# HengyiWang/spann3r

Measured on NVIDIA H100. Metric: frames/sec (512x384, 10-frame seq) enc->mem-attn->dec->DPT, higher is better.
Workload: dtype bf16x3 (split-bf16 operands, fp32 accumulate; tf32 attention)

## Files before the change

### include/spann3r_b200.h

```cpp
#ifndef SPANN3R_B200_H_
#define SPANN3R_B200_H_

#include <stddef.h>
#include <stdint.h>

#ifdef __cplusplus
extern "C" {
#endif

#define S3R_VERSION 100

enum { S3R_EPI_PLAIN = 0, S3R_EPI_PIXSHUF = 1, S3R_EPI_QKV = 2, S3R_EPI_HEADTAIL = 3 };
enum { S3R_ACT_NONE = 0, S3R_ACT_GELU = 1, S3R_ACT_RELU = 2 };

int s3r_version(void);
int s3r_abi_sizeof(int which );
const char* s3r_last_error(void);
int s3r_device_ok(void);


int s3r_split(const float* x, int64_t ldx, void* hi, void* lo, int64_t ldp, int col0, int64_t rows, int c, int relu,
              void* stream);

int s3r_layernorm(const float* x, int64_t ldx, const float* w, const float* b, int64_t wb_group_stride,
                  int64_t rows_per_group, float eps, int64_t rows, int c, float* out, int64_t ldo, void* hi, void* lo,
                  int64_t ldp, int col0, int64_t swap_rows, void* stream);

int s3r_rope2d_inplace(float* tokens, const int64_t* pos, int64_t bn, int h, int d, int64_t stride_tok,
                       int64_t stride_head, float base, float fwd, void* stream);

int s3r_im2col_patch16(const float* img, int64_t sb, int64_t sc, int64_t sy, int64_t sx, int b, int gh, int gw,
                       void* hi, void* lo, void* stream);
int s3r_im2col_3x3s2(const void* ihi, const void* ilo, int nb, int h, int w, int c, int ho, int wo, void* ohi,
                     void* olo, void* stream);
int s3r_upsample2x(const float* x, int nb, int h, int w, int c, float* out, void* hi, void* lo, void* stream);

size_t s3r_conv_wgrad_workspace_bytes(int nb, int h, int w, int n, int kc, int taps);
int s3r_conv_wgrad(const void* dy_hi, const void* dy_lo, int64_t ldy, const void* x_hi, const void* x_lo, int64_t ldx,
                   int nb, int h, int w, int n, int kc, int taps, void* workspace, size_t workspace_bytes, float* dw,
                   void* stream);
int s3r_col2im_3x3s2(const float* cols, int nb, int h, int w, int c, int ho, int wo, float* out, void* stream);

typedef struct s3r_gemm_desc {
  const void* a_hi; const void* a_lo;
  const void* b_hi; const void* b_lo;
  int groups, nb, h, w, kc, taps, n;
  int epi, act, plane_relu, force_bn;
  const float* bias;
  const float* res1; int64_t ldr1;
  const float* res2; int64_t ldr2;
  float* out_f32; int64_t ldo;
  void* out_hi; void* out_lo; int64_t ldp; int plane_col0;
  int ps_s, ps_cout;
  int q_c, q_role_base, q_ntok, q_ntok_pad, q_rope, q_nb;
  const int32_t* q_pos; const float* q_cs;
  float* q_out; float* k_out; float* vt_out; float q_scale;
  const float* ht_w; const float* ht_b; float* ht_pts; float* ht_conf;
  const float* ln_stats; int ln_np; float ln_eps; const float* ln_cs; int a_swap;
  float* stats_out;
  uint64_t* trace;
  int swap_col0; float* k2_out; float* vt2_out;
  int precision;
} s3r_gemm_desc;
int s3r_gemm(const s3r_gemm_desc* d, void* stream);
int s3r_gemm_tile_n(const s3r_gemm_desc* d);

int s3r_attention(const float* q, const float* k, const float* vt, int bh, int heads, int nq, int nk, int nk_pad,
                  void* o_hi, void* o_lo, float* o_f32, int64_t ldo, void* stream);

int s3r_conf_score(const float* conf, int64_t n, float* scratch256, float* out, void* stream);
int s3r_conf_score_batched(const float* conf, int batch, int64_t hw, float* scratch, float* out, void* stream);

int s3r_resample_h_u8(const uint8_t* src, int64_t row_stride, int rows, int out_cols, const int32_t* bounds,
                      const int32_t* kk, int ksize, int max_span, uint8_t* dst, void* stream);
int s3r_resample_v_u8_norm(const uint8_t* tmp, int cols, int out_rows, const int32_t* bounds, const int32_t* kk, int ksize,
                           float* dst, void* stream);

int s3r_focal_weiszfeld(const float* pts3d, int b, int h, int w, float ppx, float ppy, int iters, float lo, float hi,
                        float* scratch, float* focal, void* stream);

int s3r_focal_median(const float* pts3d, int b, int h, int w, float ppx, float ppy, float lo, float hi, int32_t* scratch,
                     float* focal, void* stream);

size_t s3r_pnp_workspace_bytes(int b, int n_samples);
int s3r_pnp_ransac(const float* pts3d, const float* img_pts, int b, int64_t n, int width, double fx, double fy, double cx,
                   double cy, float reproj_err, int n_samples, int refine_iters, uint64_t seed, void* workspace,
                   double* out, uint8_t* inlier_mask, void* stream);

size_t s3r_pcl_index_bytes(int64_t n);
int s3r_pcl_index_build(const void* pts, int is_f64, int64_t n, const double* transform, void* index, void* stream);
int s3r_pcl_nearest(const void* index, int64_t n, const void* queries, int is_f64, int64_t nq, const double* transform,
                    double max_dist, double* dist, int64_t* idx, void* stream);
int s3r_pcl_normals(const void* index, int64_t n, int k, double* normals, void* stream);
size_t s3r_pcl_icp_workspace_bytes(void);
int s3r_pcl_icp(const void* source, int is_f64, int64_t ns, const void* target_index, int64_t nt,
                double max_correspondence_distance, const double* init, int max_iteration, double relative_fitness,
                double relative_rmse, void* workspace, double* out, void* stream);
size_t s3r_pcl_stats_workspace_bytes(void);
int s3r_pcl_stats(const double* x, int64_t n, double threshold, void* workspace, double* out, void* stream);
int s3r_pcl_abs_dot(const double* a, const double* b, const int64_t* idx, int64_t n, double* out, void* stream);

size_t s3r_render_workspace_bytes(int width, int height);
int s3r_render_clear(void* keys, int width, int height, void* stream);
int s3r_render_splat(const float* pts, const uint8_t* mask, int64_t n, int64_t id0, const double* camera, double z_near,
                     int width, int height, void* keys, void* stream);
int s3r_render_resolve(const void* keys, const float* colors, int width, int height, uint8_t* rgb, void* stream);

typedef struct s3r_loss_desc {
  int frames, batch, height, width;
  int norm_mode, gt_scale, fix_first, shift_inv, scale_inv, conf_loss, has_dist_clip;
  float alpha, dist_clip;
  const float* pose0;
  const float* const* gt_pts;
  const uint8_t* const* valid;
  const float* const* pred;
  const float* const* conf;
} s3r_loss_desc;
#define S3R_LOSS_RES_HEADER 20
#define S3R_LOSS_RES_PER_B 6
size_t s3r_loss_workspace_bytes(const s3r_loss_desc* d);
int s3r_loss_forward(const s3r_loss_desc* d, void* workspace, size_t workspace_bytes, float* gt_out, float* pred_out,
// ... 99 lines not shown
```

### spann3r_b200/_lib.py

```python
from __future__ import annotations

import ctypes as C
import os

import torch

_HERE = os.path.dirname(os.path.abspath(__file__))
LIB_PATH = os.environ.get("S3R_LIB", os.path.join(_HERE, "libspann3r_b200.so"))

EPI_PLAIN, EPI_PIXSHUF, EPI_QKV, EPI_HEADTAIL = 0, 1, 2, 3
PRECISION_SPLIT, PRECISION_BF16 = 0, 1
ACT_NONE, ACT_GELU, ACT_RELU = 0, 1, 2

_vp, _i, _i64, _f = C.c_void_p, C.c_int, C.c_int64, C.c_float


class GemmDesc(C.Structure):
    _fields_ = [
        ("a_hi", _vp), ("a_lo", _vp), ("b_hi", _vp), ("b_lo", _vp),
        ("groups", _i), ("nb", _i), ("h", _i), ("w", _i), ("kc", _i), ("taps", _i), ("n", _i),
        ("epi", _i), ("act", _i), ("plane_relu", _i), ("force_bn", _i),
        ("bias", _vp),
        ("res1", _vp), ("ldr1", _i64),
        ("res2", _vp), ("ldr2", _i64),
        ("out_f32", _vp), ("ldo", _i64),
        ("out_hi", _vp), ("out_lo", _vp), ("ldp", _i64), ("plane_col0", _i),
        ("ps_s", _i), ("ps_cout", _i),
        ("q_c", _i), ("q_role_base", _i), ("q_ntok", _i), ("q_ntok_pad", _i), ("q_rope", _i), ("q_nb", _i),
        ("q_pos", _vp), ("q_cs", _vp),
        ("q_out", _vp), ("k_out", _vp), ("vt_out", _vp), ("q_scale", _f),
        ("ht_w", _vp), ("ht_b", _vp), ("ht_pts", _vp), ("ht_conf", _vp),
        ("ln_stats", _vp), ("ln_np", _i), ("ln_eps", _f), ("ln_cs", _vp), ("a_swap", _i),
        ("stats_out", _vp),
        ("trace", _vp),
        ("swap_col0", _i), ("k2_out", _vp), ("vt2_out", _vp),
        ("precision", _i),
    ]


class LossDesc(C.Structure):
    _fields_ = [
        ("frames", _i), ("batch", _i), ("height", _i), ("width", _i),
        ("norm_mode", _i), ("gt_scale", _i), ("fix_first", _i), ("shift_inv", _i), ("scale_inv", _i), ("conf_loss", _i),
        ("has_dist_clip", _i), ("alpha", _f), ("dist_clip", _f),
        ("pose0", _vp), ("gt_pts", C.POINTER(_vp)), ("valid", C.POINTER(_vp)), ("pred", C.POINTER(_vp)),
        ("conf", C.POINTER(_vp)),
    ]


LOSS_RES_HEADER, LOSS_RES_PER_B = 20, 6


class AttnTrainDesc(C.Structure):
    _fields_ = [
        ("batch", _i), ("heads", _i), ("nq", _i), ("nk", _i), ("dh", _i), ("scale", _f),
        ("q", _vp), ("k", _vp), ("v", _vp),
        ("q_stride", _i64 * 3), ("k_stride", _i64 * 3), ("v_stride", _i64 * 3),
    ]

_PROTOS = {
    "s3r_version": (_i, []),
    "s3r_abi_sizeof": (_i, [_i]),
    "s3r_last_error": (C.c_char_p, []),
    "s3r_device_ok": (_i, []),
    "s3r_split": (_i, [_vp, _i64, _vp, _vp, _i64, _i, _i64, _i, _i, _vp]),
    "s3r_layernorm": (_i, [_vp, _i64, _vp, _vp, _i64, _i64, _f, _i64, _i, _vp, _i64, _vp, _vp, _i64, _i, _i64, _vp]),
    "s3r_rope2d_inplace": (_i, [_vp, _vp, _i64, _i, _i, _i64, _i64, _f, _f, _vp]),
    "s3r_im2col_patch16": (_i, [_vp, _i64, _i64, _i64, _i64, _i, _i, _i, _vp, _vp, _vp]),
    "s3r_im2col_3x3s2": (_i, [_vp, _vp, _i, _i, _i, _i, _i, _i, _vp, _vp, _vp]),
    "s3r_upsample2x": (_i, [_vp, _i, _i, _i, _i, _vp, _vp, _vp, _vp]),
    "s3r_conv_wgrad_workspace_bytes": (C.c_size_t, [_i, _i, _i, _i, _i, _i]),
    "s3r_conv_wgrad": (_i, [_vp, _vp, _i64, _vp, _vp, _i64, _i, _i, _i, _i, _i, _i, _vp, C.c_size_t, _vp, _vp]),
    "s3r_col2im_3x3s2": (_i, [_vp, _i, _i, _i, _i, _i, _i, _vp, _vp]),
    "s3r_gemm": (_i, [C.POINTER(GemmDesc), _vp]),
    "s3r_gemm_tile_n": (_i, [C.POINTER(GemmDesc)]),
    "s3r_attention": (_i, [_vp, _vp, _vp, _i, _i, _i, _i, _i, _vp, _vp, _vp, _i64, _vp]),
    "s3r_conf_score": (_i, [_vp, _i64, _vp, _vp, _vp]),
    "s3r_conf_score_batched": (_i, [_vp, _i, _i64, _vp, _vp, _vp]),
    "s3r_dropout_mask": (_i, [_vp, _i64, C.c_uint64, _f, _vp]),
    "s3r_set_option": (_i, [C.c_char_p, _i]),
    "s3r_focal_weiszfeld": (_i, [_vp, _i, _i, _i, _f, _f, _i, _f, _f, _vp, _vp, _vp]),
    "s3r_focal_median": (_i, [_vp, _i, _i, _i, _f, _f, _f, _f, _vp, _vp, _vp]),
    "s3r_pnp_workspace_bytes": (C.c_size_t, [_i, _i]),
    "s3r_pnp_ransac": (_i, [_vp, _vp, _i, _i64, _i, C.c_double, C.c_double, C.c_double, C.c_double, _f, _i, _i, C.c_uint64,
                            _vp, _vp, _vp, _vp]),
    "s3r_pcl_index_bytes": (C.c_size_t, [_i64]),
    "s3r_pcl_index_build": (_i, [_vp, _i, _i64, _vp, _vp, _vp]),
    "s3r_pcl_nearest": (_i, [_vp, _i64, _vp, _i, _i64, _vp, C.c_double, _vp, _vp, _vp]),
    "s3r_pcl_normals": (_i, [_vp, _i64, _i, _vp, _vp]),
    "s3r_pcl_icp_workspace_bytes": (C.c_size_t, []),
    "s3r_pcl_icp": (_i, [_vp, _i, _i64, _vp, _i64, C.c_double, _vp, _i, C.c_double, C.c_double, _vp, _vp, _vp]),
    "s3r_pcl_stats_workspace_bytes": (C.c_size_t, []),
    "s3r_pcl_stats": (_i, [_vp, _i64, C.c_double, _vp, _vp, _vp]),
    "s3r_pcl_abs_dot": (_i, [_vp, _vp, _vp, _i64, _vp, _vp]),
    "s3r_render_workspace_bytes": (C.c_size_t, [_i, _i]),
    "s3r_render_clear": (_i, [_vp, _i, _i, _vp]),
    "s3r_render_splat": (_i, [_vp, _vp, _i64, _i64, _vp, C.c_double, _i, _i, _vp, _vp]),
    "s3r_render_resolve": (_i, [_vp, _vp, _i, _i, _vp, _vp]),
    "s3r_loss_workspace_bytes": (C.c_size_t, [C.POINTER(LossDesc)]),
    "s3r_loss_forward": (_i, [C.POINTER(LossDesc), _vp, C.c_size_t, _vp, _vp, _vp, _vp, _vp]),
    "s3r_loss_backward": (_i, [C.POINTER(LossDesc), _vp, C.c_size_t, _vp, _vp, _vp, _vp]),
    "s3r_attn_train_workspace_bytes": (C.c_size_t, [C.POINTER(AttnTrainDesc)]),
    "s3r_attn_train_forward": (_i, [C.POINTER(AttnTrainDesc), _vp, _vp, _vp]),
    "s3r_attn_train_backward": (_i, [C.POINTER(AttnTrainDesc), _vp, _vp, _vp, _vp, C.c_size_t, _vp, _vp, _vp, _vp]),
    "s3r_resample_h_u8": (_i, [_vp, _i64, _i, _i, _vp, _vp, _i, _i, _vp, _vp]),
    "s3r_resample_v_u8_norm": (_i, [_vp, _i, _i, _vp, _vp, _i, _vp, _vp]),
}

_lib = None


class S3RError(RuntimeError):
    pass


def lib():
    global _lib
    if _lib is None:
        if not os.path.exists(LIB_PATH):
            raise S3RError(f"{LIB_PATH} not found: run `python -m spann3r_b200.build` "
                           "(the package has no CPU / eager fallback)")
        L = C.CDLL(LIB_PATH)
        for name, (res, args) in _PROTOS.items():
            fn = getattr(L, name)
            fn.restype = res
            fn.argtypes = args
        _ENGINE_PROTOS_HOOK(L)
        _lib = L
    return _lib
# ... 162 lines not shown
```

### spann3r_b200/csrc/attention.cu

```cuda
#include "common.cuh"
#include "kernels.cuh"
#include "wgmma.cuh"

#include <cstdlib>
#include <cstring>

namespace s3r {

namespace attn {
constexpr int BQ = 128;
constexpr int BKV = 128;
constexpr int D = 64;
constexpr int Q_BYTES = BQ * D * 4;
constexpr int K_BYTES = BKV * D * 4;
constexpr int V_BYTES = D * BKV * 4;
constexpr int KV_STAGES = 3;
constexpr int SMEM = Q_BYTES + KV_STAGES * (K_BYTES + V_BYTES) + 1024 + 256;
constexpr int kThreads = 384;
constexpr int kConsumerWarps = 8;
}

__global__ void __launch_bounds__(attn::kThreads, 1) attention_kernel(const __grid_constant__ AttnArgs args) {
  using namespace attn;
  extern __shared__ uint8_t smem_raw[];
  uint8_t* smem = smem_raw + ((1024u - (smem_u32(smem_raw) & 1023u)) & 1023u);
  uint8_t* sQ = smem;
  uint8_t* sKV = sQ + Q_BYTES;
  uint64_t* bars = reinterpret_cast<uint64_t*>(sKV + KV_STAGES * (K_BYTES + V_BYTES));
  uint64_t* q_full = bars;
  uint64_t* kv_full = bars + 1;
  uint64_t* kv_empty = bars + 1 + KV_STAGES;

  const int warp = threadIdx.x >> 5, lane = threadIdx.x & 31;
  const int q0 = blockIdx.x * BQ;
  const int bh = blockIdx.y;
  const int nblk = (args.nk + BKV - 1) / BKV;

  if (warp == 0 && lane == 0) {
    tma_prefetch_desc(&args.tmQ);
    tma_prefetch_desc(&args.tmK);
    tma_prefetch_desc(&args.tmV);
    mbar_init(q_full, 1);
    for (int i = 0; i < KV_STAGES; ++i) {
      mbar_init(&kv_full[i], 1);
      mbar_init(&kv_empty[i], kConsumerWarps);
    }
    fence_barrier_init();
  }
  __syncthreads();
  pdl_launch_dependents();
  pdl_wait();

  if (warp < 4) {
    asm volatile("setmaxnreg.dec.sync.aligned.u32 40;");
    if (warp == 0 && lane == 0) {
      mbar_arrive_expect_tx(q_full, Q_BYTES);
      tma_load_3d(sQ, &args.tmQ, q_full, 0, q0, bh);
      tma_load_3d(sQ + Q_BYTES / 2, &args.tmQ, q_full, 32, q0, bh);
      for (int j = 0; j < nblk; ++j) {
        const int st = j % KV_STAGES;
        const uint32_t ph = (j / KV_STAGES) & 1;
        mbar_wait(&kv_empty[st], ph ^ 1);
        uint8_t* k = sKV + st * (K_BYTES + V_BYTES);
        uint8_t* v = k + K_BYTES;
        mbar_arrive_expect_tx(&kv_full[st], K_BYTES + V_BYTES);
        tma_load_3d(k, &args.tmK, &kv_full[st], 0, j * BKV, bh);
        tma_load_3d(k + K_BYTES / 2, &args.tmK, &kv_full[st], 32, j * BKV, bh);
#pragma unroll
        for (int a = 0; a < 4; ++a) tma_load_3d(v + a * (V_BYTES / 4), &args.tmV, &kv_full[st], j * BKV + a * 32, 0, bh);
      }
    }
    return;
  }

  asm volatile("setmaxnreg.inc.sync.aligned.u32 232;");
  const int wg = (warp - 4) >> 2;
  const int wq = warp & 3;
  const int g = lane >> 2, t4 = lane & 3;
  const uint32_t aQ = __shfl_sync(0xffffffffu, smem_u32(sQ), 0) + wg * (64 * 128);
  const uint32_t aKV = __shfl_sync(0xffffffffu, smem_u32(sKV), 0);
  constexpr float kLog2e = 1.4426950408889634f;

  float o[32];
#pragma unroll
  for (int i = 0; i < 32; ++i) o[i] = 0.f;
  float m0 = -INFINITY, m1 = -INFINITY, l0 = 0.f, l1 = 0.f;
  const int src_lo = (lane & ~3) | (t4 >> 1), src_hi = src_lo + 2;
  const bool odd = (t4 & 1) != 0;

  mbar_wait(q_full, 0);
  for (int j = 0; j < nblk; ++j) {
    const int st = j % KV_STAGES;
    mbar_wait(&kv_full[st], (j / KV_STAGES) & 1);
    const uint32_t aK = aKV + st * (K_BYTES + V_BYTES);
    const uint32_t aV = aK + K_BYTES;

    float s[64];
    wgmma_fence();
#pragma unroll
    for (int kk = 0; kk < 8; ++kk) {
      const uint32_t part = (kk >> 2) * (Q_BYTES / 2), ko = (kk & 3) * 2;
      wgmma_tf32_n128_ss(s, wgmma_desc_sw128_kmajor(aQ + part) + ko, wgmma_desc_sw128_kmajor(aK + part) + ko, kk > 0);
    }
    wgmma_commit();
    wgmma_wait<0>();

    const int kbase = j * BKV;
    if (kbase + BKV > args.nk) {
#pragma unroll
      for (int i = 0; i < 16; ++i) {
        const int c = kbase + 8 * i + 2 * t4;
        if (c >= args.nk) { s[4 * i] = -INFINITY; s[4 * i + 2] = -INFINITY; }
        if (c + 1 >= args.nk) { s[4 * i + 1] = -INFINITY; s[4 * i + 3] = -INFINITY; }
      }
    }
    float b0 = -INFINITY, b1 = -INFINITY;
#pragma unroll
    for (int i = 0; i < 16; ++i) {
      b0 = fmaxf(b0, fmaxf(s[4 * i], s[4 * i + 1]));
      b1 = fmaxf(b1, fmaxf(s[4 * i + 2], s[4 * i + 3]));
    }
#pragma unroll
    for (int x = 1; x < 4; x <<= 1) {
      b0 = fmaxf(b0, __shfl_xor_sync(0xffffffffu, b0, x));
      b1 = fmaxf(b1, __shfl_xor_sync(0xffffffffu, b1, x));
    }
    const float n0 = fmaxf(m0, b0), n1 = fmaxf(m1, b1);
    const float al0 = (j == 0) ? 0.f : exp2f((m0 - n0) * kLog2e);
    const float al1 = (j == 0) ? 0.f : exp2f((m1 - n1) * kLog2e);
    m0 = n0;
    m1 = n1;
    const float nr0 = -n0 * kLog2e, nr1 = -n1 * kLog2e;
    float ps0 = 0.f, ps1 = 0.f;
#pragma unroll
    for (int i = 0; i < 64; ++i) {
      const bool r1 = (i & 2) != 0;
      const float e = exp2f(fmaf(s[i], kLog2e, r1 ? nr1 : nr0));
      const uint32_t rb = (__float_as_uint(e) + 0x1000u) & 0xffffe000u;
      s[i] = __uint_as_float(rb);
      if (r1) ps1 += s[i]; else ps0 += s[i];
    }
    l0 = l0 * al0 + ps0;
    l1 = l1 * al1 + ps1;
#pragma unroll
    for (int i = 0; i < 8; ++i) {
      o[4 * i] *= al0; o[4 * i + 1] *= al0;
      o[4 * i + 2] *= al1; o[4 * i + 3] *= al1;
    }

    uint32_t pa[16][4];
#pragma unroll
    for (int kk = 0; kk < 16; ++kk) {
      const float x0 = __shfl_sync(0xffffffffu, s[4 * kk], src_lo), x1 = __shfl_sync(0xffffffffu, s[4 * kk + 1], src_lo);
      const float y0 = __shfl_sync(0xffffffffu, s[4 * kk + 2], src_lo), y1 = __shfl_sync(0xffffffffu, s[4 * kk + 3], src_lo);
      const float z0 = __shfl_sync(0xffffffffu, s[4 * kk], src_hi), z1 = __shfl_sync(0xffffffffu, s[4 * kk + 1], src_hi);
      const float w0 = __shfl_sync(0xffffffffu, s[4 * kk + 2], src_hi), w1 = __shfl_sync(0xffffffffu, s[4 * kk + 3], src_hi);
      pa[kk][0] = __float_as_uint(odd ? x1 : x0);
      pa[kk][1] = __float_as_uint(odd ? y1 : y0);
      pa[kk][2] = __float_as_uint(odd ? z1 : z0);
      pa[kk][3] = __float_as_uint(odd ? w1 : w0);
    }
    wgmma_fence();
#pragma unroll
    for (int kk = 0; kk < 16; ++kk)
      wgmma_tf32_n64_rs(o, pa[kk], wgmma_desc_sw128_kmajor(aV + (kk >> 2) * (V_BYTES / 4)) + (kk & 3) * 2, 1);
    wgmma_commit();
    wgmma_wait<0>();
    __syncwarp();
    if (lane == 0) mbar_arrive(&kv_empty[st]);
  }

#pragma unroll
  for (int x = 1; x < 4; x <<= 1) {
    l0 += __shfl_xor_sync(0xffffffffu, l0, x);
    l1 += __shfl_xor_sync(0xffffffffu, l1, x);
  }
  const float inv0 = 1.0f / l0, inv1 = 1.0f / l1;
  const int b = bh / args.heads, h = bh - b * args.heads;
#pragma unroll
  for (int r = 0; r < 2; ++r) {
    const int q = q0 + wg * 64 + wq * 16 + g + 8 * r;
    if (q >= args.nq) continue;
    const float inv = r ? inv1 : inv0;
    const long long row = ((long long)b * args.nq + q) * args.ldo + h * D;
#pragma unroll
    for (int i = 0; i < 8; ++i) {
      const float x = o[4 * i + 2 * r] * inv, y = o[4 * i + 2 * r + 1] * inv;
      const long long off = row + 8 * i + 2 * t4;
      if (args.o_f32) *reinterpret_cast<float2*>(args.o_f32 + off) = make_float2(x, y);
      if (args.o_hi) {
        uint32_t hh, ll;
        split2_bf16(x, y, hh, ll);
        *reinterpret_cast<uint32_t*>(args.o_hi + off) = hh;
        *reinterpret_cast<uint32_t*>(args.o_lo + off) = ll;
      }
    }
  }
}

int attn_plan_init(AttnPlan* plan, const float* q, const float* k, const float* vt, int BH, int heads, int nq, int nk,
                   int nk_pad) {
  using namespace attn;
  memset(plan, 0, sizeof(*plan));
  if (nk_pad % 4 != 0 || nk_pad < nk) {
    set_error("attention: nk_pad=%d must be >= nk=%d and a multiple of 4", nk_pad, nk);
    return -1;
  }
  AttnArgs& a = plan->args;
  {
    uint64_t dims[3] = {64, (uint64_t)nq, (uint64_t)BH};
    uint64_t str[2] = {64 * 4, (uint64_t)nq * 64 * 4};
    uint32_t box[3] = {32, (uint32_t)BQ, 1};
    int r = encode_tmap(&a.tmQ, CU_TENSOR_MAP_DATA_TYPE_FLOAT32, 3, q, dims, str, box);
    if (r) return r;
  }
  {
    uint64_t dims[3] = {64, (uint64_t)nk, (uint64_t)BH};
    uint64_t str[2] = {64 * 4, (uint64_t)nk * 64 * 4};
    uint32_t box[3] = {32, (uint32_t)BKV, 1};
    int r = encode_tmap(&a.tmK, CU_TENSOR_MAP_DATA_TYPE_FLOAT32, 3, k, dims, str, box);
    if (r) return r;
  }
  {
    uint64_t dims[3] = {(uint64_t)nk, 64, (uint64_t)BH};
    uint64_t str[2] = {(uint64_t)nk_pad * 4, (uint64_t)nk_pad * 64 * 4};
    uint32_t box[3] = {32, 64, 1};
    int r = encode_tmap(&a.tmV, CU_TENSOR_MAP_DATA_TYPE_FLOAT32, 3, vt, dims, str, box);
    if (r) return r;
  }
  a.nq = nq; a.nk = nk; a.heads = heads;
  plan->grid = dim3((nq + BQ - 1) / BQ, BH);
  plan->flops = 4.0 * BH * (double)nq * nk * 64;
  return 0;
}

static int attn_launch_args(const AttnPlan& plan, const AttnArgs& a, cudaStream_t st) {
  using namespace attn;
  static PerDeviceOnce once;
  bool& attr_set = once.cur();
  if (!attr_set) {
    cudaError_t e = cudaFuncSetAttribute(attention_kernel, cudaFuncAttributeMaxDynamicSharedMemorySize, SMEM);
    if (e != cudaSuccess) {
      set_error("attention: cudaFuncSetAttribute(smem=%d): %s", SMEM, cudaGetErrorString(e));
      return -5;
    }
    attr_set = true;
  }
  cudaError_t e = launch_pdl(attention_kernel, plan.grid, dim3(kThreads), SMEM, st, a);
  if (e != cudaSuccess) {
    set_error("attention launch failed: %s", cudaGetErrorString(e));
    return -6;
  }
  return 0;
}

int attn_launch(const AttnPlan& plan, __nv_bfloat16* o_hi, __nv_bfloat16* o_lo, float* o_f32, long long ldo,
                cudaStream_t st) {
  AttnArgs a = plan.args;
  a.o_hi = o_hi; a.o_lo = o_lo; a.o_f32 = o_f32; a.ldo = ldo;
  return attn_launch_args(plan, a, st);
}

int launch_attention(const float* q, const float* k, const float* vt, int BH, int heads, int nq, int nk, int nk_pad,
                     __nv_bfloat16* o_hi, __nv_bfloat16* o_lo, float* o_f32, long long ldo, cudaStream_t st) {
  if (heads <= 0 || BH % heads != 0 || ldo % 2 != 0) {
    set_error("attention: bh=%d must be a multiple of heads=%d, and ldo=%lld even (paired stores)", BH, heads, ldo);
    return -1;
  }
  if (nq <= 0 || nk <= 0 || BH <= 0) return 0;
  AttnPlan plan;
  int r = attn_plan_init(&plan, q, k, vt, BH, heads, nq, nk, nk_pad);
  if (r) return r;
  return attn_launch(plan, o_hi, o_lo, o_f32, ldo, st);
}

}
```

### spann3r_b200/csrc/capi.cu

```cuda
#include "../../include/spann3r_b200.h"

#include <cstring>

#include "gemm.cuh"
#include "kernels.cuh"

using namespace s3r;

static inline cudaStream_t S(void* s) { return reinterpret_cast<cudaStream_t>(s); }
static inline __nv_bfloat16* B(void* p) { return reinterpret_cast<__nv_bfloat16*>(p); }
static inline const __nv_bfloat16* B(const void* p) { return reinterpret_cast<const __nv_bfloat16*>(p); }

extern "C" {

int s3r_version(void) { return S3R_VERSION; }
int s3r_abi_sizeof(int which) {
  switch (which) {
    case 0: return (int)sizeof(s3r_gemm_desc);
    case 1: return (int)sizeof(s3r_model_w);
    case 2: return (int)sizeof(s3r_bank);
    case 3: return (int)sizeof(s3r_loss_desc);
    case 4: return (int)sizeof(s3r_attn_train_desc);
  }
  return -1;
// ... 245 lines not shown
  return launch_pcl_icp(source, is_f64, ns, target_index, nt, max_correspondence_distance, init, max_iteration,
                        relative_fitness, relative_rmse, workspace, out, S(stream));
}
size_t s3r_pcl_stats_workspace_bytes(void) { return pcl_stats_workspace_bytes(); }
int s3r_pcl_stats(const double* x, int64_t n, double threshold, void* workspace, double* out, void* stream) {
  return launch_pcl_stats(x, n, threshold, workspace, out, S(stream));
}
int s3r_pcl_abs_dot(const double* a, const double* b, const int64_t* idx, int64_t n, double* out, void* stream) {
  return launch_pcl_abs_dot(a, b, reinterpret_cast<const long long*>(idx), n, out, S(stream));
}

size_t s3r_render_workspace_bytes(int width, int height) { return render_workspace_bytes(width, height); }
int s3r_render_clear(void* keys, int width, int height, void* stream) {
  return launch_render_clear(keys, width, height, S(stream));
}
int s3r_render_splat(const float* pts, const uint8_t* mask, int64_t n, int64_t id0, const double* camera, double z_near,
                     int width, int height, void* keys, void* stream) {
  return launch_render_splat(pts, mask, n, id0, camera, z_near, width, height, keys, S(stream));
}
int s3r_render_resolve(const void* keys, const float* colors, int width, int height, uint8_t* rgb, void* stream) {
  return launch_render_resolve(keys, colors, width, height, rgb, S(stream));
}

size_t s3r_loss_workspace_bytes(const s3r_loss_desc* d) { return loss_workspace_bytes(d); }
int s3r_loss_forward(const s3r_loss_desc* d, void* workspace, size_t workspace_bytes, float* gt_out, float* pred_out,
                     uint8_t* valid_out, double* results, void* stream) {
  return launch_loss_forward(d, workspace, workspace_bytes, gt_out, pred_out, valid_out, results, S(stream));
}
int s3r_loss_backward(const s3r_loss_desc* d, const void* workspace, size_t workspace_bytes, const float* upstream,
                      float* grad_pred, float* grad_conf, void* stream) {
  return launch_loss_backward(d, workspace, workspace_bytes, upstream, grad_pred, grad_conf, S(stream));
}

size_t s3r_attn_train_workspace_bytes(const s3r_attn_train_desc* d) { return attn_train_workspace_bytes(d); }
int s3r_attn_train_forward(const s3r_attn_train_desc* d, float* o, float* lse, void* stream) {
  return launch_attn_train_forward(d, o, lse, S(stream));
}
int s3r_attn_train_backward(const s3r_attn_train_desc* d, const float* o, const float* lse, const float* d_o,
                            void* workspace, size_t workspace_bytes, float* dq, float* dk, float* dv, void* stream) {
  return launch_attn_train_backward(d, o, lse, d_o, workspace, workspace_bytes, dq, dk, dv, S(stream));
}

int s3r_conf_score(const float* conf, int64_t n, float* scratch256, float* out, void* stream) {
  return launch_conf_score(conf, n, scratch256, out, S(stream));
}
int s3r_conf_score_batched(const float* conf, int batch, int64_t hw, float* scratch, float* out, void* stream) {
  return launch_conf_score_batched(conf, batch, hw, scratch, out, S(stream));
}

int s3r_set_option(const char* name, int value) {
  s3r::Options& o = s3r::options();
  if (!name) { set_error("s3r_set_option: null name"); return -1; }
  if (!strcmp(name, "prefetch_b")) o.prefetch_b = value;
  else { set_error("s3r_set_option: unknown option '%s' (prefetch_b)", name); return -1; }
  return 0;
}

int s3r_dropout_mask(float* out, int64_t n, uint64_t seed, float p, void* stream) {
  if (!out && n > 0) {
    set_error("s3r_dropout_mask: null output");
    return -1;
  }
  return launch_dropout_mask(out, n, seed, p, S(stream));
}

int s3r_attention(const float* q, const float* k, const float* vt, int bh, int heads, int nq, int nk, int nk_pad,
                  void* o_hi, void* o_lo, float* o_f32, int64_t ldo, void* stream) {
  return launch_attention(q, k, vt, bh, heads, nq, nk, nk_pad, B(o_hi), B(o_lo), o_f32, ldo, S(stream));
}

}
```

### spann3r_b200/csrc/common.cuh

```cuda
#pragma once
#include <cuda.h>
#include <cuda_bf16.h>
#include <cuda_runtime.h>
#include <stdint.h>

#include <cstdlib>
#include <utility>

namespace s3r {

__device__ __forceinline__ uint32_t smem_u32(const void* p) {
  return static_cast<uint32_t>(__cvta_generic_to_shared(p));
}
__device__ __forceinline__ uint32_t lane_id() { return threadIdx.x & 31; }
__device__ __forceinline__ bool elect_one() {
  uint32_t pred = 0;
  asm volatile(
      "{\n\t.reg .pred P1;\n\t"
      "elect.sync _|P1, 0xffffffff;\n\t"
      "selp.u32 %0, 1, 0, P1;\n\t}\n"
      : "=r"(pred));
  return pred != 0;
}

// ... 34 lines not shown
  asm volatile("mbarrier.arrive.expect_tx.shared::cta.b64 _, [%0], %1;" ::"r"(smem_u32(bar)), "r"(bytes)
               : "memory");
}
__device__ __forceinline__ void mbar_arrive(uint64_t* bar) {
  asm volatile("mbarrier.arrive.shared::cta.b64 _, [%0];" ::"r"(smem_u32(bar)) : "memory");
}
__device__ __forceinline__ bool mbar_try_wait(uint64_t* bar, uint32_t parity) {
  uint32_t ok;
  asm volatile(
      "{\n\t.reg .pred P1;\n\t"
      "mbarrier.try_wait.parity.shared::cta.b64 P1, [%1], %2;\n\t"
      "selp.u32 %0, 1, 0, P1;\n\t}\n"
      : "=r"(ok)
      : "r"(smem_u32(bar)), "r"(parity)
      : "memory");
  return ok != 0;
}
__device__ __forceinline__ void mbar_wait(uint64_t* bar, uint32_t parity) {
  uint32_t spins = 0;
  while (!mbar_try_wait(bar, parity)) {
    if (++spins > (1u << 28)) { asm volatile("trap;"); }
  }
}

__device__ __forceinline__ void fence_proxy_async_smem() {
  asm volatile("fence.proxy.async.shared::cta;" ::: "memory");
}
__device__ __forceinline__ void tma_prefetch_desc(const CUtensorMap* m) {
  asm volatile("prefetch.tensormap [%0];" ::"l"(reinterpret_cast<uint64_t>(m)) : "memory");
}
__device__ __forceinline__ void tma_load_2d(void* smem, const CUtensorMap* m, uint64_t* bar, int c0, int c1) {
  asm volatile(
      "cp.async.bulk.tensor.2d.shared::cta.global.mbarrier::complete_tx::bytes [%0], [%1, {%3, %4}], [%2];" ::"r"(
          smem_u32(smem)),
      "l"(reinterpret_cast<uint64_t>(m)), "r"(smem_u32(bar)), "r"(c0), "r"(c1)
      : "memory");
}
__device__ __forceinline__ void tma_load_3d(void* smem, const CUtensorMap* m, uint64_t* bar, int c0, int c1,
                                            int c2) {
  asm volatile(
      "cp.async.bulk.tensor.3d.shared::cta.global.mbarrier::complete_tx::bytes [%0], [%1, {%3, %4, %5}], [%2];" ::
          "r"(smem_u32(smem)),
      "l"(reinterpret_cast<uint64_t>(m)), "r"(smem_u32(bar)), "r"(c0), "r"(c1), "r"(c2)
      : "memory");
}
__device__ __forceinline__ void tma_load_4d(void* smem, const CUtensorMap* m, uint64_t* bar, int c0, int c1,
                                            int c2, int c3) {
  asm volatile(
      "cp.async.bulk.tensor.4d.shared::cta.global.mbarrier::complete_tx::bytes [%0], [%1, {%3, %4, %5, %6}], "
      "[%2];" ::"r"(smem_u32(smem)),
      "l"(reinterpret_cast<uint64_t>(m)), "r"(smem_u32(bar)), "r"(c0), "r"(c1), "r"(c2), "r"(c3)
      : "memory");
}

__device__ __forceinline__ void mbar_arrive_expect_tx_u(uint32_t bar, uint32_t bytes) {
  asm volatile("mbarrier.arrive.expect_tx.shared::cta.b64 _, [%0], %1;" ::"r"(bar), "r"(bytes) : "memory");
}
__device__ __forceinline__ void tma_load_3d_u(uint32_t smem, const CUtensorMap* m, uint32_t bar, int c0, int c1, int c2) {
  asm volatile(
      "cp.async.bulk.tensor.3d.shared::cta.global.mbarrier::complete_tx::bytes [%0], [%1, {%3, %4, %5}], [%2];" ::
          "r"(smem),
      "l"(reinterpret_cast<uint64_t>(m)), "r"(bar), "r"(c0), "r"(c1), "r"(c2)
      : "memory");
}
__device__ __forceinline__ void tma_load_4d_u(uint32_t smem, const CUtensorMap* m, uint32_t bar, int c0, int c1, int c2,
                                              int c3) {
  asm volatile(
      "cp.async.bulk.tensor.4d.shared::cta.global.mbarrier::complete_tx::bytes [%0], [%1, {%3, %4, %5, %6}], "
      "[%2];" ::"r"(smem),
      "l"(reinterpret_cast<uint64_t>(m)), "r"(bar), "r"(c0), "r"(c1), "r"(c2), "r"(c3)
      : "memory");
}

__device__ __forceinline__ uint64_t wgmma_desc_sw128_kmajor(uint32_t smem_addr) {
  uint64_t d = 0;
  d |= (uint64_t)((smem_addr & 0x3FFFF) >> 4);
  d |= (uint64_t)1 << 16;
  d |= (uint64_t)64 << 32;
  d |= (uint64_t)1 << 62;
  return d;
}

__device__ __forceinline__ uint64_t wgmma_desc_sw64_kmajor(uint32_t smem_addr) {
  uint64_t d = 0;
  d |= (uint64_t)((smem_addr & 0x3FFFF) >> 4);
  d |= (uint64_t)1 << 16;
  d |= (uint64_t)32 << 32;
  d |= (uint64_t)2 << 62;
  return d;
}

__device__ __forceinline__ void pdl_launch_dependents() { asm volatile("griddepcontrol.launch_dependents;" ::: "memory"); }
__device__ __forceinline__ void pdl_wait() { asm volatile("griddepcontrol.wait;" ::: "memory"); }

__device__ __forceinline__ unsigned long long globaltimer_ns() {
  unsigned long long t;
  asm volatile("mov.u64 %0, %%globaltimer;" : "=l"(t));
  return t;
}

__device__ __forceinline__ void st_f4(float* p, float a, float b, float c, float d) {
  *reinterpret_cast<float4*>(p) = make_float4(a, b, c, d);
}

struct PerDeviceOnce {
  bool done[64] = {};
// ... 25 lines not shown
```

### spann3r_b200/csrc/gemm.cuh

```cuda
#pragma once
#include <cuda.h>
#include <cuda_bf16.h>
#include <cuda_runtime.h>
#include <stdint.h>

namespace s3r {

enum EpiMode : int {
  EPI_PLAIN = 0,
  EPI_PIXSHUF = 1,
  EPI_QKV = 2,
  EPI_HEADTAIL = 3,
};
enum Act : int { ACT_NONE = 0, ACT_GELU = 1, ACT_RELU = 2 };
enum GemmPrecision : int { GEMM_SPLIT = 0, GEMM_BF16 = 1 };

struct GemmArgs {
  alignas(64) CUtensorMap tmA_hi;
  alignas(64) CUtensorMap tmA_lo;
  alignas(64) CUtensorMap tmB_hi;
  alignas(64) CUtensorMap tmB_lo;
  int groups;
  int W, H, NB;
  int bw, bh;
  int tiles_w, tiles_h;
  int N;
  int Kc, taps, kpt;
  int b_group_rows;
  int epi, act, plane_relu;
  const float* bias;
  const float* res1; int ldr1;
  const float* res2; int ldr2;
  float* out_f32; int ldo;
  __nv_bfloat16* out_hi; __nv_bfloat16* out_lo; int ldp; int plane_col0;
  long long out_group_rows;
  const float2* ln_stats; int ln_np; float ln_eps;
  const float* ln_cs;
  int b_static;
  int a_swap;
  int swap_col0;
  float2* stats_out;
  unsigned long long* trace;
  int ps_s, ps_cout;
  int q_C, q_role_base, q_ntok, q_ntok_pad, q_rope, q_nb;
  const int* q_pos;
  const float2* q_cs;
  float* q_out; float* k_out; float* vt_out;
  float* k2_out; float* vt2_out;
  float q_scale;
  const float* ht_w;
  const float* ht_b;
  float* ht_pts;
  float* ht_conf;
};

struct GemmPlan {
  GemmArgs args;
  dim3 grid;
  int bn;
  int precision;
  int b_static;
  double flops;
};

int gemm_plan_init(GemmPlan* plan,
                   const __nv_bfloat16* a_hi, const __nv_bfloat16* a_lo,
                   const __nv_bfloat16* b_hi, const __nv_bfloat16* b_lo,
                   int groups, int NB, int H, int W, int Kc, int taps, int N, int force_bn = 0,
                   long long lda = 0, long long ldb = 0, long long b_group_rows = 0, int precision = GEMM_SPLIT);
int gemm_launch(const GemmPlan& plan, cudaStream_t stream);

struct Options {
  int prefetch_b = 1;
};
Options& options();
int num_sms();

int encode_tmap(CUtensorMap* out, CUtensorMapDataType dt, int rank, const void* base, const uint64_t* dims,
                const uint64_t* strides_bytes, const uint32_t* box,
                CUtensorMapSwizzle swizzle = CU_TENSOR_MAP_SWIZZLE_128B);
const char* last_error();
void set_error(const char* fmt, ...);

}
```

### spann3r_b200/csrc/kernels.cuh

```cuda
#pragma once
#include <cuda_bf16.h>
#include <cuda_runtime.h>

#include "gemm.cuh"
#include <cuda.h>

struct s3r_loss_desc;
struct s3r_attn_train_desc;

namespace s3r {

int launch_split(const float* x, long long ldx, __nv_bfloat16* hi, __nv_bfloat16* lo, long long ldp, int col0,
                 long long rows, int C, int relu, cudaStream_t st);
int launch_split_stats(const float* x, long long ldx, long long rows, int C, float* out, long long ldo, __nv_bfloat16* hi,
                       __nv_bfloat16* lo, long long ldp, float2* stats, cudaStream_t st);
int launch_layernorm(const float* x, long long ldx, const float* w, const float* b, long long wb_group_stride,
                     long long rows_per_group, float eps, long long rows, int C, float* out, long long ldo,
                     __nv_bfloat16* hi, __nv_bfloat16* lo, long long ldp, int col0, long long swap_rows,
                     cudaStream_t st);
int launch_im2col_patch16(const float* img, long long sb, long long sc, long long sy, long long sx, int B, int gh,
                          int gw, __nv_bfloat16* hi, __nv_bfloat16* lo, cudaStream_t st);
int launch_im2col_3x3s2(const __nv_bfloat16* ihi, const __nv_bfloat16* ilo, int NB, int H, int W, int C, int Ho, int Wo,
                        __nv_bfloat16* ohi, __nv_bfloat16* olo, cudaStream_t st);
int launch_upsample2x(const float* x, int NB, int H, int W, int C, float* out, __nv_bfloat16* hi, __nv_bfloat16* lo,
                      cudaStream_t st, int Ho = 0, int Wo = 0);
int launch_rope2d(float* tokens, const long long* pos, long long BN, int H, int D, long long stride_tok,
                  long long stride_head, float base, float fwd, cudaStream_t st);

struct AttnArgs {
  alignas(64) CUtensorMap tmQ;
  alignas(64) CUtensorMap tmK;
  alignas(64) CUtensorMap tmV;
  int nq, nk, heads;
  __nv_bfloat16* o_hi;
  __nv_bfloat16* o_lo;
  float* o_f32;
  long long ldo;
};
struct AttnPlan {
  AttnArgs args;
  dim3 grid;
  double flops;
};
int attn_plan_init(AttnPlan* plan, const float* q, const float* k, const float* vt, int BH, int heads, int nq, int nk,
                   int nk_pad);
int attn_launch(const AttnPlan& plan, __nv_bfloat16* o_hi, __nv_bfloat16* o_lo, float* o_f32, long long ldo,
                cudaStream_t st);

constexpr int MEM_SOFTMAX_MAX_LEN = 200 * 1024 / 4;
constexpr int MEM_MAX_SLOTS = 64;
struct SlotInts {
  int n;
  int v[MEM_MAX_SLOTS];
  __host__ __device__ int operator[](int b) const { return v[n == 1 ? 0 : b]; }
};
inline SlotInts slot_uniform(int x) { SlotInts s{}; s.n = 1; s.v[0] = x; return s; }
int launch_mem_softmax(const float* S, long long ldS, long long rows, int nq, const SlotInts& lens, int Mmax, int Mpad,
                       float scale, float thresh, __nv_bfloat16* phi, __nv_bfloat16* plo, long long ldP, cudaStream_t st,
                       float drop_p = 0.f, unsigned long long seed = 0);
int launch_dropout_mask(float* out, long long n, unsigned long long seed, float p, cudaStream_t st);
int launch_mem_colsum(const __nv_bfloat16* phi, const __nv_bfloat16* plo, long long ldP, int B, int nq, const SlotInts& lens,
                      int Mmax, float* mem_attn, long long ld_attn, float* part, long long ld_part, cudaStream_t st);
int launch_split_transpose(const float* x, int B, int T, int C, __nv_bfloat16* ohi, __nv_bfloat16* olo, long long ldo,
                           long long out_batch_stride, const SlotInts& col0, const SlotInts& on, cudaStream_t st);
int launch_check_sim(const float* feat, const float* k, long long k_batch_stride, int B, const SlotInts& start,
                     const SlotInts& wm, int P, int C, float* scratch, float* out, int ldo, cudaStream_t st);

int launch_resample_h_u8(const uint8_t* src, long long row_stride, int rows, int out_cols, const int* bounds,
                         const int* kk, int ksize, int max_span, uint8_t* dst, cudaStream_t st);
int launch_resample_v_u8_norm(const uint8_t* tmp, int cols, int out_rows, const int* bounds, const int* kk, int ksize,
                              float* dst, cudaStream_t st);

int launch_focal_weiszfeld(const float* pts3d, int B, int H, int W, float ppx, float ppy, int iters, float lo, float hi,
                           float* scratch, float* focal, cudaStream_t st);

size_t pnp_workspace_bytes(int B, int n_samples);
int launch_pnp_ransac(const float* pts3d, const float* img_pts, int B, long long n, int width, double fx, double fy,
                      double cx, double cy, float reproj_err, int n_samples, int refine_iters, unsigned long long seed,
                      void* workspace, double* out, unsigned char* inlier_mask, cudaStream_t st);

int launch_focal_median(const float* pts3d, int B, int H, int W, float ppx, float ppy, float lo, float hi, int* scratch,
                        float* focal, cudaStream_t st);

int launch_conf_score(const float* conf, long long n, float* scratch256, float* out, cudaStream_t st);
int launch_conf_score_batched(const float* conf, int batch, long long hw, float* scratch, float* out, cudaStream_t st);

size_t pcl_index_bytes(long long n);
int launch_pcl_index_build(const void* pts, int f64, long long n, const double* T, void* index, cudaStream_t st);
int launch_pcl_nearest(const void* index, long long n, const void* q, int f64, long long nq, const double* T,
                       double max_dist, double* dist, long long* idx, cudaStream_t st);
int launch_pcl_normals(const void* index, long long n, int k, double* normals, cudaStream_t st);
size_t pcl_icp_workspace_bytes();
int launch_pcl_icp(const void* src, int f64, long long ns, const void* target_index, long long nt, double max_corr,
                   const double* init, int max_iteration, double rel_fitness, double rel_rmse, void* workspace,
                   double* out, cudaStream_t st);
size_t pcl_stats_workspace_bytes();
// ... 31 lines not shown
```

Measured before the change: 88.59.

## Add permuted-K TMA layout and 192-row query tile to attention kernel

Templates the attention kernel on the number of consumer warpgroups (128 or 192 query rows per CTA). It also adds a rank-5 TMA view of K that permutes key columns so the P accumulator fragments feed the PV wgmma directly without warp shuffles. A planner picks the 192-row tile when a wave-quantization cost model favours it, and the softmax/PV loop is split into two halves to overlap exp with wgmma. The cost is more register pressure, fewer KV stages for the 3-warpgroup variant, and an approximate ex2 on the permuted path.

```diff
diff --git a/include/spann3r_b200.h b/include/spann3r_b200.h
--- a/include/spann3r_b200.h
+++ b/include/spann3r_b200.h
@@ -67,6 +67,7 @@
 
 int s3r_attention(const float* q, const float* k, const float* vt, int bh, int heads, int nq, int nk, int nk_pad,
                   void* o_hi, void* o_lo, float* o_f32, int64_t ldo, void* stream);
+int s3r_attention_tile(int bh, int nq, int nk, int num_sms, int attn_bq, int attn_kperm, int* out);
 
 int s3r_conf_score(const float* conf, int64_t n, float* scratch256, float* out, void* stream);
 int s3r_conf_score_batched(const float* conf, int batch, int64_t hw, float* scratch, float* out, void* stream);
diff --git a/spann3r_b200/_lib.py b/spann3r_b200/_lib.py
--- a/spann3r_b200/_lib.py
+++ b/spann3r_b200/_lib.py
@@ -75,6 +75,7 @@
     "s3r_gemm": (_i, [C.POINTER(GemmDesc), _vp]),
     "s3r_gemm_tile_n": (_i, [C.POINTER(GemmDesc)]),
     "s3r_attention": (_i, [_vp, _vp, _vp, _i, _i, _i, _i, _i, _vp, _vp, _vp, _i64, _vp]),
+    "s3r_attention_tile": (_i, [_i, _i, _i, _i, _i, _i, C.POINTER(_i)]),
     "s3r_conf_score": (_i, [_vp, _i64, _vp, _vp, _vp]),
     "s3r_conf_score_batched": (_i, [_vp, _i, _i64, _vp, _vp, _vp]),
     "s3r_dropout_mask": (_i, [_vp, _i64, C.c_uint64, _f, _vp]),
diff --git a/spann3r_b200/csrc/attention.cu b/spann3r_b200/csrc/attention.cu
--- a/spann3r_b200/csrc/attention.cu
+++ b/spann3r_b200/csrc/attention.cu
@@ -2,26 +2,41 @@
 #include "kernels.cuh"
 #include "wgmma.cuh"
 
+#include <cstdio>
 #include <cstdlib>
 #include <cstring>
 
 namespace s3r {
 
 namespace attn {
-constexpr int BQ = 128;
 constexpr int BKV = 128;
 constexpr int D = 64;
-constexpr int Q_BYTES = BQ * D * 4;
 constexpr int K_BYTES = BKV * D * 4;
 constexpr int V_BYTES = D * BKV * 4;
-constexpr int KV_STAGES = 3;
-constexpr int SMEM = Q_BYTES + KV_STAGES * (K_BYTES + V_BYTES) + 1024 + 256;
-constexpr int kThreads = 384;
-constexpr int kConsumerWarps = 8;
-}
-
-__global__ void __launch_bounds__(attn::kThreads, 1) attention_kernel(const __grid_constant__ AttnArgs args) {
+template <int NC>
+struct Tile {
+  static constexpr int BQ = 64 * NC;
+  static constexpr int Q_BYTES = BQ * D * 4;
+  static constexpr int STAGES = NC == 2 ? 3 : 2;
+  static constexpr int SMEM = Q_BYTES + STAGES * (K_BYTES + V_BYTES) + 1024 + 256;
+  static constexpr int THREADS = 128 * (NC + 1);
+  static constexpr int CONSUMER_WARPS = 4 * NC;
+  static constexpr int CONSUMER_REGS = NC == 2 ? 232 : 152;
+};
+}
+
+__device__ __forceinline__ float ex2_ftz(float x) {
+  float y;
+  asm("ex2.approx.ftz.f32 %0, %1;" : "=f"(y) : "f"(x));
+  return y;
+}
+
+template <int NC, bool KPERM>
+__global__ void __launch_bounds__(attn::Tile<NC>::THREADS, 1) attention_kernel(const __grid_constant__ AttnArgs args) {
   using namespace attn;
+  using T = Tile<NC>;
+  constexpr int BQ = T::BQ, Q_BYTES = T::Q_BYTES, KV_STAGES = T::STAGES;
+  static_assert(NC == 2 || KPERM, "the shuffle path's P copy does not fit the 3-warpgroup register budget");
   extern __shared__ uint8_t smem_raw[];
   uint8_t* smem = smem_raw + ((1024u - (smem_u32(smem_raw) & 1023u)) & 1023u);
   uint8_t* sQ = smem;
@@ -43,7 +58,7 @@
     mbar_init(q_full, 1);
     for (int i = 0; i < KV_STAGES; ++i) {
       mbar_init(&kv_full[i], 1);
-      mbar_init(&kv_empty[i], kConsumerWarps);
+      mbar_init(&kv_empty[i], T::CONSUMER_WARPS);
     }
     fence_barrier_init();
   }
@@ -64,8 +79,13 @@
         uint8_t* k = sKV + st * (K_BYTES + V_BYTES);
         uint8_t* v = k + K_BYTES;
         mbar_arrive_expect_tx(&kv_full[st], K_BYTES + V_BYTES);
-        tma_load_3d(k, &args.tmK, &kv_full[st], 0, j * BKV, bh);
-        tma_load_3d(k + K_BYTES / 2, &args.tmK, &kv_full[st], 32, j * BKV, bh);
+        if constexpr (KPERM) {
+          tma_load_5d(k, &args.tmK, &kv_full[st], 0, 0, 0, j * (BKV / 8), bh);
+          tma_load_5d(k + K_BYTES / 2, &args.tmK, &kv_full[st], 32, 0, 0, j * (BKV / 8), bh);
+        } else {
+          tma_load_3d(k, &args.tmK, &kv_full[st], 0, j * BKV, bh);
+          tma_load_3d(k + K_BYTES / 2, &args.tmK, &kv_full[st], 32, j * BKV, bh);
+        }
 #pragma unroll
         for (int a = 0; a < 4; ++a) tma_load_3d(v + a * (V_BYTES / 4), &args.tmV, &kv_full[st], j * BKV + a * 32, 0, bh);
       }
@@ -73,11 +93,11 @@
     return;
   }
 
-  asm volatile("setmaxnreg.inc.sync.aligned.u32 232;");
+  asm volatile("setmaxnreg.inc.sync.aligned.u32 %0;" ::"n"(T::CONSUMER_REGS));
   const int wg = (warp - 4) >> 2;
   const int wq = warp & 3;
   const int g = lane >> 2, t4 = lane & 3;
-  const uint32_t aQ = __shfl_sync(0xffffffffu, smem_u32(sQ), 0) + wg * (64 * 128);
+  const uint32_t aQ = __shfl_sync(0xffffffffu, smem_u32(sQ) + wg * (64 * 128), 0);
   const uint32_t aKV = __shfl_sync(0xffffffffu, smem_u32(sKV), 0);
   constexpr float kLog2e = 1.4426950408889634f;
 
@@ -99,8 +119,8 @@
     wgmma_fence();
 #pragma unroll
     for (int kk = 0; kk < 8; ++kk) {
-      const uint32_t part = (kk >> 2) * (Q_BYTES / 2), ko = (kk & 3) * 2;
-      wgmma_tf32_n128_ss(s, wgmma_desc_sw128_kmajor(aQ + part) + ko, wgmma_desc_sw128_kmajor(aK + part) + ko, kk > 0);
+      const uint32_t part = (kk >> 2) * (Q_BYTES / 2), kpart = (kk >> 2) * (K_BYTES / 2), ko = (kk & 3) * 2;
+      wgmma_tf32_n128_ss(s, wgmma_desc_sw128_kmajor(aQ + part) + ko, wgmma_desc_sw128_kmajor(aK + kpart) + ko, kk > 0);
     }
     wgmma_commit();
     wgmma_wait<0>();
@@ -109,9 +129,9 @@
     if (kbase + BKV > args.nk) {
 #pragma unroll
       for (int i = 0; i < 16; ++i) {
-        const int c = kbase + 8 * i + 2 * t4;
+        const int c = kbase + 8 * i + (KPERM ? t4 : 2 * t4);
         if (c >= args.nk) { s[4 * i] = -INFINITY; s[4 * i + 2] = -INFINITY; }
-        if (c + 1 >= args.nk) { s[4 * i + 1] = -INFINITY; s[4 * i + 3] = -INFINITY; }
+        if (c + (KPERM ? 4 : 1) >= args.nk) { s[4 * i + 1] = -INFINITY; s[4 * i + 3] = -INFINITY; }
       }
     }
     float b0 = -INFINITY, b1 = -INFINITY;
@@ -131,40 +151,51 @@
     m0 = n0;
     m1 = n1;
     const float nr0 = -n0 * kLog2e, nr1 = -n1 * kLog2e;
-    float ps0 = 0.f, ps1 = 0.f;
-#pragma unroll
-    for (int i = 0; i < 64; ++i) {
-      const bool r1 = (i & 2) != 0;
-      const float e = exp2f(fmaf(s[i], kLog2e, r1 ? nr1 : nr0));
-      const uint32_t rb = (__float_as_uint(e) + 0x1000u) & 0xffffe000u;
-      s[i] = __uint_as_float(rb);
-      if (r1) ps1 += s[i]; else ps0 += s[i];
-    }
-    l0 = l0 * al0 + ps0;
-    l1 = l1 * al1 + ps1;
 #pragma unroll
     for (int i = 0; i < 8; ++i) {
       o[4 * i] *= al0; o[4 * i + 1] *= al0;
       o[4 * i + 2] *= al1; o[4 * i + 3] *= al1;
     }
 
+    float ps0 = 0.f, ps1 = 0.f;
     uint32_t pa[16][4];
 #pragma unroll
-    for (int kk = 0; kk < 16; ++kk) {
-      const float x0 = __shfl_sync(0xffffffffu, s[4 * kk], src_lo), x1 = __shfl_sync(0xffffffffu, s[4 * kk + 1], src_lo);
-      const float y0 = __shfl_sync(0xffffffffu, s[4 * kk + 2], src_lo), y1 = __shfl_sync(0xffffffffu, s[4 * kk + 3], src_lo);
-      const float z0 = __shfl_sync(0xffffffffu, s[4 * kk], src_hi), z1 = __shfl_sync(0xffffffffu, s[4 * kk + 1], src_hi);
-      const float w0 = __shfl_sync(0xffffffffu, s[4 * kk + 2], src_hi), w1 = __shfl_sync(0xffffffffu, s[4 * kk + 3], src_hi);
-      pa[kk][0] = __float_as_uint(odd ? x1 : x0);
-      pa[kk][1] = __float_as_uint(odd ? y1 : y0);
-      pa[kk][2] = __float_as_uint(odd ? z1 : z0);
-      pa[kk][3] = __float_as_uint(odd ? w1 : w0);
-    }
-    wgmma_fence();
-#pragma unroll
-    for (int kk = 0; kk < 16; ++kk)
-      wgmma_tf32_n64_rs(o, pa[kk], wgmma_desc_sw128_kmajor(aV + (kk >> 2) * (V_BYTES / 4)) + (kk & 3) * 2, 1);
-    wgmma_commit();
+    for (int hf = 0; hf < 2; ++hf) {
+#pragma unroll
+      for (int i = 32 * hf; i < 32 * hf + 32; ++i) {
+        const bool r1 = (i & 2) != 0;
+        const float x = fmaf(s[i], kLog2e, r1 ? nr1 : nr0);
+        const float e = KPERM ? ex2_ftz(x) : exp2f(x);
+        const uint32_t rb = (__float_as_uint(e) + 0x1000u) & 0xffffe000u;
+        s[i] = __uint_as_float(rb);
+        if (r1) ps1 += s[i]; else ps0 += s[i];
+      }
+#pragma unroll
+      for (int kk = 8 * hf; kk < 8 * hf + 8; ++kk) {
+        if constexpr (KPERM) {
+          pa[kk][0] = __float_as_uint(s[4 * kk]);
+          pa[kk][1] = __float_as_uint(s[4 * kk + 2]);
+          pa[kk][2] = __float_as_uint(s[4 * kk + 1]);
+          pa[kk][3] = __float_as_uint(s[4 * kk + 3]);
+        } else {
+          const float x0 = __shfl_sync(0xffffffffu, s[4 * kk], src_lo), x1 = __shfl_sync(0xffffffffu, s[4 * kk + 1], src_lo);
+          const float y0 = __shfl_sync(0xffffffffu, s[4 * kk + 2], src_lo), y1 = __shfl_sync(0xffffffffu, s[4 * kk + 3], src_lo);
+          const float z0 = __shfl_sync(0xffffffffu, s[4 * kk], src_hi), z1 = __shfl_sync(0xffffffffu, s[4 * kk + 1], src_hi);
+          const float w0 = __shfl_sync(0xffffffffu, s[4 * kk + 2], src_hi), w1 = __shfl_sync(0xffffffffu, s[4 * kk + 3], src_hi);
+          pa[kk][0] = __float_as_uint(odd ? x1 : x0);
+          pa[kk][1] = __float_as_uint(odd ? y1 : y0);
+          pa[kk][2] = __float_as_uint(odd ? z1 : z0);
+          pa[kk][3] = __float_as_uint(odd ? w1 : w0);
+        }
+      }
+      wgmma_fence();
+#pragma unroll
+      for (int kk = 8 * hf; kk < 8 * hf + 8; ++kk)
+        wgmma_tf32_n64_rs(o, pa[kk], wgmma_desc_sw128_kmajor(aV + (kk >> 2) * (V_BYTES / 4)) + (kk & 3) * 2, 1);
+      wgmma_commit();
+    }
+    l0 = l0 * al0 + ps0;
+    l1 = l1 * al1 + ps1;
     wgmma_wait<0>();
     __syncwarp();
     if (lane == 0) mbar_arrive(&kv_empty[st]);
@@ -198,6 +229,34 @@
   }
 }
 
+int attn_pick_tile(int BH, int nq, int nk, int sms, int force_bq, int force_kperm, int* bq, int* kperm) {
+  if (BH <= 0 || nq <= 0 || nk <= 0 || sms <= 0) {
+    set_error("attention tile: bh=%d, nq=%d, nk=%d and sms=%d must be positive", BH, nq, nk, sms);
+    return -1;
+  }
+  if ((force_bq != 0 && force_bq != 128 && force_bq != 192) || force_kperm < -1 || force_kperm > 1) {
+    set_error("attention tile: attn_bq=%d (0, 128 or 192), attn_kperm=%d (-1, 0 or 1)", force_bq, force_kperm);
+    return -1;
+  }
+  const bool perm_ok = nk % 8 == 0;
+  if (force_kperm == 1 && !perm_ok) {
+    set_error("attention tile: attn_kperm=1 needs nk %% 8 == 0 (nk=%d)", nk);
+    return -1;
+  }
+  if (force_bq == 192 && (force_kperm == 0 || !perm_ok)) {
+    set_error("attention tile: attn_bq=192 runs on the permuted K only (attn_kperm=%d, nk=%d)", force_kperm, nk);
+    return -1;
+  }
+  *kperm = force_kperm >= 0 ? force_kperm : (perm_ok ? 1 : 0);
+  if (force_bq) {
+    *bq = force_bq;
+    return 0;
+  }
+  auto cost = [&](int t) { return (long long)(((long long)(nq + t - 1) / t * BH + sms - 1) / sms) * t; };
+  *bq = (*kperm && cost(192) < cost(128)) ? 192 : 128;
+  return 0;
+}
+
 int attn_plan_init(AttnPlan* plan, const float* q, const float* k, const float* vt, int BH, int heads, int nq, int nk,
                    int nk_pad) {
   using namespace attn;
@@ -206,15 +265,30 @@
     set_error("attention: nk_pad=%d must be >= nk=%d and a multiple of 4", nk_pad, nk);
     return -1;
   }
+  const Options& opt = options();
+  int bq = 0, kperm = 0;
+  if (int r = attn_pick_tile(BH, nq, nk, 1, opt.attn_bq, opt.attn_kperm, &bq, &kperm)) return r;
+  if (opt.attn_bq == 0) attn_pick_tile(BH, nq, nk, num_sms(), opt.attn_bq, opt.attn_kperm, &bq, &kperm);
   AttnArgs& a = plan->args;
   {
     uint64_t dims[3] = {64, (uint64_t)nq, (uint64_t)BH};
     uint64_t str[2] = {64 * 4, (uint64_t)nq * 64 * 4};
-    uint32_t box[3] = {32, (uint32_t)BQ, 1};
+    uint32_t box[3] = {32, (uint32_t)bq, 1};
     int r = encode_tmap(&a.tmQ, CU_TENSOR_MAP_DATA_TYPE_FLOAT32, 3, q, dims, str, box);
     if (r) return r;
   }
-  {
+  if (kperm) {
+    uint64_t dims[5] = {64, 2, 4, (uint64_t)nk / 8, (uint64_t)BH};
+    uint64_t str[4] = {4 * 64 * 4, 64 * 4, 8 * 64 * 4, (uint64_t)nk * 64 * 4};
+    uint32_t box[5] = {32, 2, 4, BKV / 8, 1};
+    if (int r = encode_tmap(&a.tmK, CU_TENSOR_MAP_DATA_TYPE_FLOAT32, 5, k, dims, str, box)) {
+      char why[256];
+      snprintf(why, sizeof(why), "%s", last_error());
+      set_error("attention: the driver rejected the rank-5 permuted view of K (nk=%d, bh=%d; attn_kperm=0 avoids it): %s",
+                nk, BH, why);
+      return r;
+    }
+  } else {
     uint64_t dims[3] = {64, (uint64_t)nk, (uint64_t)BH};
     uint64_t str[2] = {64 * 4, (uint64_t)nk * 64 * 4};
     uint32_t box[3] = {32, (uint32_t)BKV, 1};
@@ -229,29 +303,37 @@
     if (r) return r;
   }
   a.nq = nq; a.nk = nk; a.heads = heads;
-  plan->grid = dim3((nq + BQ - 1) / BQ, BH);
+  plan->bq = bq;
+  plan->kperm = kperm;
+  plan->grid = dim3((nq + bq - 1) / bq, BH);
   plan->flops = 4.0 * BH * (double)nq * nk * 64;
   return 0;
 }
 
-static int attn_launch_args(const AttnPlan& plan, const AttnArgs& a, cudaStream_t st) {
-  using namespace attn;
+template <int NC, bool KPERM>
+static int attn_launch_variant(const AttnPlan& plan, const AttnArgs& a, cudaStream_t st) {
+  using T = attn::Tile<NC>;
   static PerDeviceOnce once;
   bool& attr_set = once.cur();
   if (!attr_set) {
-    cudaError_t e = cudaFuncSetAttribute(attention_kernel, cudaFuncAttributeMaxDynamicSharedMemorySize, SMEM);
+    cudaError_t e = cudaFuncSetAttribute(attention_kernel<NC, KPERM>, cudaFuncAttributeMaxDynamicSharedMemorySize, T::SMEM);
     if (e != cudaSuccess) {
-      set_error("attention: cudaFuncSetAttribute(smem=%d): %s", SMEM, cudaGetErrorString(e));
+      set_error("attention: cudaFuncSetAttribute(smem=%d): %s", T::SMEM, cudaGetErrorString(e));
       return -5;
     }
     attr_set = true;
   }
-  cudaError_t e = launch_pdl(attention_kernel, plan.grid, dim3(kThreads), SMEM, st, a);
+  cudaError_t e = launch_pdl(attention_kernel<NC, KPERM>, plan.grid, dim3(T::THREADS), T::SMEM, st, a);
   if (e != cudaSuccess) {
     set_error("attention launch failed: %s", cudaGetErrorString(e));
     return -6;
   }
   return 0;
+}
+
+static int attn_launch_args(const AttnPlan& plan, const AttnArgs& a, cudaStream_t st) {
+  if (plan.bq == 192) return attn_launch_variant<3, true>(plan, a, st);
+  return plan.kperm ? attn_launch_variant<2, true>(plan, a, st) : attn_launch_variant<2, false>(plan, a, st);
 }
 
 int attn_launch(const AttnPlan& plan, __nv_bfloat16* o_hi, __nv_bfloat16* o_lo, float* o_f32, long long ldo,
diff --git a/spann3r_b200/csrc/capi.cu b/spann3r_b200/csrc/capi.cu
--- a/spann3r_b200/csrc/capi.cu
+++ b/spann3r_b200/csrc/capi.cu
@@ -321,8 +321,28 @@
   s3r::Options& o = s3r::options();
   if (!name) { set_error("s3r_set_option: null name"); return -1; }
   if (!strcmp(name, "prefetch_b")) o.prefetch_b = value;
-  else { set_error("s3r_set_option: unknown option '%s' (prefetch_b)", name); return -1; }
+  else if (!strcmp(name, "attn_bq")) {
+    if (value != 0 && value != 128 && value != 192) {
+      set_error("s3r_set_option: attn_bq=%d (0 = the planner's, 128, 192)", value);
+      return -1;
+    }
+    o.attn_bq = value;
+  } else if (!strcmp(name, "attn_kperm")) {
+    if (value < -1 || value > 1) {
+      set_error("s3r_set_option: attn_kperm=%d (-1 = the planner's, 0, 1)", value);
+      return -1;
+    }
+    o.attn_kperm = value;
+  } else {
+    set_error("s3r_set_option: unknown option '%s' (prefetch_b, attn_bq, attn_kperm)", name);
+    return -1;
+  }
   return 0;
+}
+
+int s3r_attention_tile(int bh, int nq, int nk, int num_sms, int attn_bq, int attn_kperm, int* out) {
+  if (!out) { set_error("s3r_attention_tile: null output"); return -1; }
+  return attn_pick_tile(bh, nq, nk, num_sms, attn_bq, attn_kperm, &out[0], &out[1]);
 }
 
 int s3r_dropout_mask(float* out, int64_t n, uint64_t seed, float p, void* stream) {
diff --git a/spann3r_b200/csrc/common.cuh b/spann3r_b200/csrc/common.cuh
--- a/spann3r_b200/csrc/common.cuh
+++ b/spann3r_b200/csrc/common.cuh
@@ -110,6 +110,14 @@
       "l"(reinterpret_cast<uint64_t>(m)), "r"(smem_u32(bar)), "r"(c0), "r"(c1), "r"(c2), "r"(c3)
       : "memory");
 }
+__device__ __forceinline__ void tma_load_5d(void* smem, const CUtensorMap* m, uint64_t* bar, int c0, int c1,
+                                            int c2, int c3, int c4) {
+  asm volatile(
+      "cp.async.bulk.tensor.5d.shared::cta.global.mbarrier::complete_tx::bytes [%0], [%1, {%3, %4, %5, %6, %7}], "
+      "[%2];" ::"r"(smem_u32(smem)),
+      "l"(reinterpret_cast<uint64_t>(m)), "r"(smem_u32(bar)), "r"(c0), "r"(c1), "r"(c2), "r"(c3), "r"(c4)
+      : "memory");
+}
 
 __device__ __forceinline__ void mbar_arrive_expect_tx_u(uint32_t bar, uint32_t bytes) {
   asm volatile("mbarrier.arrive.expect_tx.shared::cta.b64 _, [%0], %1;" ::"r"(bar), "r"(bytes) : "memory");
diff --git a/spann3r_b200/csrc/gemm.cuh b/spann3r_b200/csrc/gemm.cuh
--- a/spann3r_b200/csrc/gemm.cuh
+++ b/spann3r_b200/csrc/gemm.cuh
@@ -72,6 +72,8 @@
 
 struct Options {
   int prefetch_b = 1;
+  int attn_bq = 0;
+  int attn_kperm = -1;
 };
 Options& options();
 int num_sms();
diff --git a/spann3r_b200/csrc/kernels.cuh b/spann3r_b200/csrc/kernels.cuh
--- a/spann3r_b200/csrc/kernels.cuh
+++ b/spann3r_b200/csrc/kernels.cuh
@@ -39,9 +39,12 @@
 };
 struct AttnPlan {
   AttnArgs args;
+  int bq;
+  int kperm;
   dim3 grid;
   double flops;
 };
+int attn_pick_tile(int BH, int nq, int nk, int sms, int force_bq, int force_kperm, int* bq, int* kperm);
 int attn_plan_init(AttnPlan* plan, const float* q, const float* k, const float* vt, int BH, int heads, int nq, int nk,
                    int nk_pad);
 int attn_launch(const AttnPlan& plan, __nv_bfloat16* o_hi, __nv_bfloat16* o_lo, float* o_f32, long long ldo,
```

New measurement: 90.90, median of 6. 1.03x the previous value.
